# robocin/rSoccer

Hardware: AMD Instinct MI355X
Metric: env-steps/sec (whole node), VSS-v0 3v3 @4096 envs, 1/2/4/8 GPU + CPU ref (higher is better)
Workload: dtype f32

## Files before the change

rsoccer_amd/csrc/rsx_api.hip:

```cpp
#include <hip/hip_runtime.h>

#include <cstdio>
#include <cmath>
#include <cstdlib>
#include <algorithm>
#include <cstring>
#include <string>
#include <vector>

#include "rsx.h"
#include "rsx_units.hpp"
#include "rsx_variants.hpp"

using namespace rsx;

namespace {

thread_local std::string g_err;

int fail(int code, const std::string& msg) { g_err = msg; return code; }

#define HIP_TRY(expr)                                                                      \
    do {                                                                                   \
        hipError_t _e = (expr);                                                            \
// ... 591 lines not shown
    RSX_ENTER(h);
    h->host_state_valid = false;
    launch_sim(h, (hipStream_t)stream);
    HIP_TRY(launch_status());
    return debug_finite(h, (hipStream_t)stream, "rsx_step_dev");
}

static int ensure_alt(rsx_sim* h) {
    if (h->d_state_alt) return RSX_OK;
    const size_t sbytes = (size_t)(h->P.state_dim + X_ROWS) * h->P.row_stride * sizeof(float);
    HIP_TRY(hipMalloc((void**)&h->alt_alloc, sbytes));
    h->d_state_alt = h->alt_alloc;
    HIP_TRY(hipMemset(h->d_state_alt, 0, sbytes));
    HIP_TRY(hipDeviceSynchronize());
    return RSX_OK;
}

int rsx_state_buffers(rsx_sim* h, float** current, float** other) {
    RSX_ENTER(h);
    if (!current || !other) return fail(RSX_ERR_ARG, "null argument");
    if (int rc = ensure_alt(h)) return rc;
    *current = h->d_state; *other = h->d_state_alt;
    h->host_state_cache = false; h->host_state_valid = false;
    return RSX_OK;
}

int rsx_step_dev_random(rsx_sim* h, int n, uint64_t seed, uint32_t first_tick, void* stream) {
    RSX_ENTER(h);
    if (n < 1) return fail(RSX_ERR_ARG, "n must be >= 1");
    if ((uint64_t)first_tick + (uint64_t)n > 0x7FFFFFFFull) return fail(RSX_ERR_ARG, "tick range exceeds 2^31");
    h->host_state_valid = false;
    for (int i = 0; i < n; ++i) launch_sim(h, (hipStream_t)stream, nullptr, (int)(first_tick + (uint32_t)i), seed);
    HIP_TRY(launch_status());
    return debug_finite(h, (hipStream_t)stream, "rsx_step_dev_random");
}

int rsx_step_dev_flip(rsx_sim* h, void* stream) {
    RSX_ENTER(h);
    {
        hipStreamCaptureStatus cs = hipStreamCaptureStatusNone;
        if (hipStreamIsCapturing((hipStream_t)stream, &cs) != hipSuccess) (void)hipGetLastError();
        else if (cs != hipStreamCaptureStatusNone) return fail(RSX_ERR_STATE, "rsx_step_dev_flip cannot be captured (the buffer roles are host state); capture rsx_step_dev instead");
    }
    if (int rc = ensure_alt(h)) return rc;
    h->host_state_valid = false;
    launch_sim(h, (hipStream_t)stream, h->d_state_alt);
    HIP_TRY(launch_status());
    std::swap(h->d_state, h->d_state_alt);
    return debug_finite(h, (hipStream_t)stream, "rsx_step_dev_flip");
}

int rsx_reset_dev(rsx_sim* h, const float* ball_dev, const float* blue_dev, const float* yellow_dev,
                  const uint8_t* env_mask_dev, void* stream) {
    RSX_ENTER(h);
    if (!ball_dev || (h->P.n_blue && !blue_dev) || (h->P.n_yellow && !yellow_dev)) return fail(RSX_ERR_ARG, "null placement array");
    h->host_state_valid = false;
    const int B = h->P.num_envs;
    rsx_launch(reset_dev_kernel, dim3((B + 255) / 256), dim3(256), 0, (hipStream_t)stream, h->d_state, ball_dev, blue_dev,
                       yellow_dev, env_mask_dev, B, h->P.row_stride, h->P.state_dim + X_ROWS, h->M.rs, h->P.n_blue, h->P.n_yellow, (float)h->M.field[6]);
    HIP_TRY(launch_status());
    return RSX_OK;
}

int rsx_task_attach(rsx_sim* h, int task, uint64_t seed, uint64_t env_id_base, int max_episode_steps) {
    RSX_ENTER(h);
    if (h->P.task != RSX_TASK_NONE) return fail(RSX_ERR_STATE, "a task is already attached");
    if (env_id_base > 0xFFFFFFFFull || env_id_base + (uint64_t)h->P.num_envs > 0x100000000ull)
        return fail(RSX_ERR_ARG, "env_id_base + num_envs exceeds 2^32 (global env ids are 32-bit)");
    Params P = h->P;
    if (derive_task(task, seed, env_id_base, max_episode_steps, h->M, P))
        return fail(RSX_ERR_ARG, "task does not match the simulator (VSS_V0: VSS, n_blue >= 1; STATIC_DEFENDERS: SSL 1vN; DRIBBLING: SSL 1v4; CONTESTED: SSL 1v1; PASS_ENDURANCE: SSL 2v0; SCRIMMAGE: SSL)");
    if (P.obs_dim > 64) return fail(RSX_ERR_ARG, "observation wider than 64 floats is not supported");
    if (task >= RSX_TASK_SSL_DRIBBLING && task <= RSX_TASK_SSL_PASS_ENDURANCE && h->L != 8)
        return fail(RSX_ERR_ARG, "this task runs with 8 lanes per env only (unset RSX_LANES_PER_ENV)");
    const size_t B = (size_t)P.num_envs, S = (size_t)P.row_stride;
    const size_t n_aux = align_up((size_t)aux_rows(P.n_robots) * S * sizeof(float));
    if (n_aux >= ((size_t)1 << 32) || B * (size_t)P.obs_dim * sizeof(float) >= ((size_t)1 << 32))
        return fail(RSX_ERR_ARG, "num_envs too large for a fused task: the per-env scalar arena or the observation array would reach 4 GB (see rsx.h, limits)");
    const size_t n_obs = align_up(B * P.obs_dim * sizeof(float));
    const size_t n_flags = align_up(3 * B);
    const size_t n_act = align_up(B * h->M.act_dim * sizeof(float));
    const size_t n_met = align_up((size_t)TICK_SLOT_WORD0 * 4 + ((size_t)grid_for(h) + (B + 63) / 64) * sizeof(uint32_t));
    const size_t n_slots = align_up((size_t)MSLOTS * RSX_METRICS * sizeof(unsigned long long));
    const bool pc = !std::getenv("RSX_NO_PCACHE") && h->L == 8 && P.num_envs <= RSX_PCACHE_MAX_ENVS && P.n_sub > 0 &&
                    task == RSX_TASK_SSL_STATIC_DEFENDERS && h->NR == 7;
    const size_t n_pc = pc ? align_up((size_t)2 * (3 * (P.n_robots + 1) + 1) * B * sizeof(float)) : 0;
    const size_t n_pcs = pc && std::getenv("RSX_PCACHE_STATS") ? align_up(2 * sizeof(unsigned long long)) : 0;
    const size_t total = n_aux + 2 * n_obs + n_flags + n_act + n_met + n_slots + n_pc + n_pcs;
    HIP_TRY(hipMalloc((void**)&h->arena_task, total));
    HIP_TRY(hipMemset(h->arena_task, 0, total));
    h->arena_task_bytes = total; h->pcache_bytes = n_pc;
    char* p = h->arena_task;
    h->d_aux = (float*)p; p += n_aux;
    h->d_obs = (float*)p; p += n_obs;
    h->d_final_obs = (float*)p; p += n_obs;
    h->d_flags = (uint8_t*)p; p += n_flags;
    h->d_actions = (float*)p; p += n_act;
    h->d_metrics = (unsigned long long*)p; p += n_met;
    h->d_mslots = (unsigned long long*)p; p += n_slots;
    if (n_pc) {
        h->d_pcache = (float*)p; p += n_pc;
        HIP_TRY(hipMemset(h->d_pcache, 0xFF, n_pc));
    }
    if (n_pcs) h->d_pcstats = (unsigned long long*)p;
    HIP_TRY(hipMemset(h->d_aux + (size_t)ROW_EPISODE * S, 0xFF, B * sizeof(uint32_t)));
    h->P = P;
    h->epl = false;
    h->big = false; h->quad = false;
    if ((task == RSX_TASK_SSL_SCRIMMAGE || task == RSX_TASK_SSL_SCRIMMAGE_CROWDED) && h->NR == 22 && h->L == 32) {
        h->big = P.num_envs >= RSX_BIG_MIN_ENVS;
        const char* lay = std::getenv("RSX_LAYOUT");
        const size_t rows = (size_t)std::max(P.state_dim + X_ROWS, aux_rows(P.n_robots));
        const bool fits = rows * (size_t)P.row_stride * sizeof(float) < ((size_t)1 << 31) && P.n_sub > 0 && P.n_blue == 11;
        const int quad_min = task == RSX_TASK_SSL_SCRIMMAGE ? RSX_QUAD_MIN_ENVS : RSX_QUAD_MIN_ENVS_CROWDED;
        h->quad = fits && (lay ? std::strcmp(lay, "quad") == 0 : (quad_min > 0 && P.num_envs >= quad_min));
    }
    const bool fixed_ssl = task == RSX_TASK_SSL_DRIBBLING || task == RSX_TASK_SSL_CONTESTED || task == RSX_TASK_SSL_PASS_ENDURANCE;
    if ((task == RSX_TASK_VSS_V0 && h->NR == 6 && h->L == 8) || (task == RSX_TASK_SSL_STATIC_DEFENDERS && h->NR == 7 && h->L == 8) || fixed_ssl) {
        const char* lay = std::getenv("RSX_LAYOUT");
        if (lay && std::strcmp(lay, "epl") == 0) h->epl = true;
        else if (lay && std::strcmp(lay, "lanes") == 0) h->epl = false;
        else h->epl = P.num_envs >= (task == RSX_TASK_VSS_V0 ? RSX_EPL_MIN_ENVS : task == RSX_TASK_SSL_STATIC_DEFENDERS ? RSX_EPL_MIN_ENVS_SSL
                                     : task == RSX_TASK_SSL_DRIBBLING ? 49152 : 32768);
        const size_t rows = (size_t)std::max(P.state_dim + X_ROWS, aux_rows(P.n_robots));
        if (rows * (size_t)P.row_stride * sizeof(float) >= ((size_t)1 << 31) || (size_t)P.num_envs * P.obs_dim * sizeof(float) >= ((size_t)1 << 31)) h->epl = false;
    }
    if (h->d_phys) h->epl = h->big = h->quad = false;
    h->task_ready = false;
    h->tick_dev = false;
    h->tick_slots = step_grid(h, MODE_STEP);
    h->tick_slots_alloc = std::max(h->tick_slots, grid_for(h) + (P.num_envs + 63) / 64);
    HIP_TRY(hipDeviceSynchronize());
    return RSX_OK;
}

int rsx_drop_pending_hip_error(void) { return (int)hipGetLastError(); }

int rsx_task_reseed(rsx_sim* h, uint64_t seed, void* stream) {
    RSX_ENTER_TASK(h);
    hipStream_t s = (hipStream_t)stream;
    hipStreamCaptureStatus cs = hipStreamCaptureStatusNone;
    if (hipStreamIsCapturing(s, &cs) != hipSuccess) (void)hipGetLastError();
    else if (cs != hipStreamCaptureStatusNone) return fail(RSX_ERR_STATE, "rsx_task_reseed changes host state (seed, step counter) and cannot be captured");
    HIP_TRY(hipMemsetAsync(h->arena_task, 0, h->arena_task_bytes, s));
    if (h->d_pcache) HIP_TRY(hipMemsetAsync(h->d_pcache, 0xFF, h->pcache_bytes, s));
    HIP_TRY(hipMemsetAsync(h->d_aux + (size_t)ROW_EPISODE * h->P.row_stride, 0xFF, (size_t)h->P.num_envs * sizeof(uint32_t), s));
    h->P.key0 = (uint32_t)seed; h->P.key1 = (uint32_t)(seed >> 32);
    h->tick = 0; h->P.tick_base = 0;
    h->task_ready = false;
    return RSX_OK;
}

int rsx_task_enable_capture(rsx_sim* h, void* stream) {
    RSX_ENTER_TASK(h);
    (void)hipGetLastError();
    if (h->tick_dev) return RSX_OK;
    hipStream_t s = (hipStream_t)stream;
    hipStreamCaptureStatus cs = hipStreamCaptureStatusNone;
    if (hipStreamIsCapturing(s, &cs) != hipSuccess) (void)hipGetLastError();
    else if (cs != hipStreamCaptureStatusNone)
        return fail(RSX_ERR_STATE, "rsx_task_enable_capture must be called BEFORE the capture begins (it writes the step counter once; a captured write would reset it on every replay)");
    tick_fill(h, 0, h->tick_slots_alloc, h->tick, 0, s);
    HIP_TRY(launch_status());
    h->tick_dev = true;
    h->host_state_cache = false; h->host_state_valid = false;
    return RSX_OK;
}

// ... 479 lines not shown
```

rsoccer_amd/csrc/rsx_kernels.hpp:

```cpp
#pragma once
#include <hip/hip_runtime.h>
#include <type_traits>

#include "rsx_math.hpp"
#include "rsx_params.hpp"
#include "rsx_body.hpp"
#include "rsx_phys.hpp"

namespace rsx {

constexpr int ROW_REWARD = 0, ROW_PREV_POT = 1, ROW_EP_RET = 2, ROW_STEPS = 3, ROW_EPISODE = 4,
              ROW_INFO = 5 , ROW_OU = 15 ;
__host__ __device__ constexpr int aux_rows(int n_robots) { return ROW_OU + 2 * n_robots; }

struct Buffers {
    float* state;
    float* aux;
    float* obs;
    float* final_obs;
    uint8_t* flags;
    const float* cmds;
    const float* actions;
    unsigned long long* metrics;
    unsigned long long* mslots;
    float* pcache;
    unsigned long long* pcstats;
#ifdef RSX_TIMING
    unsigned long long* dbg;
#endif
};

template <int L>
struct Shared {
    float4 A[64];
    float4 Bq[64];
    float4 Cq[64];
    float Dq[64];
    float W[64];
    float2 F[64];
    alignas(16) float X[64], Y[64];
    float x0[64 / L][12];
    float2 draws[64 / L][L < 16 ? 16 : L];
    uint32_t ep[64];
#ifdef RSX_TIMING
    unsigned long long* dbg;
#endif
};

#define RSX_RARE_B(KIND, bit, c) (((KIND) == RSX_KIND_SSL || (6 & (bit))) ? __builtin_expect(!!(c), 0) : !!(c))

typedef uint32_t ix_t;
__device__ __forceinline__ float& at_byte(float* base, const ix_t off) { return *reinterpret_cast<float*>(reinterpret_cast<char*>(base) + off); }
__device__ __forceinline__ const float& at_byte(const float* base, const ix_t off) { return *reinterpret_cast<const float*>(reinterpret_cast<const char*>(base) + off); }

template <int L>
struct LaneMap {
    static constexpr int G = 64 / L;
    static constexpr bool EM = L == 8;
    static __device__ __forceinline__ int slot(const int j, const int g) { return EM ? g * L + j : j * G + g; }
    static __device__ __forceinline__ int body(const int lane) { return EM ? lane % L : lane / G; }
    static __device__ __forceinline__ int env(const int lane) { return EM ? lane / L : lane % G; }
};
template <int L>
__device__ __forceinline__ unsigned long long env_lane_mask(const int g) {
    constexpr int G = 64 / L;
    if (LaneMap<L>::EM) return ((1ull << L) - 1ull) << (g * L);
    unsigned long long m = 0;
#pragma unroll
    for (int j = 0; j < L; ++j) m |= 1ull << (j * G);
    return m << g;
}

__device__ __forceinline__ void load_coefs(const Params& P, const float* __restrict__ phys, const int e, EnvCoef& cf) {
    const float* const rows = phys + PHYS_HDR_FLOATS + (size_t)NPHYS * (size_t)P.row_stride;
    const ix_t B4 = (ix_t)4 * (ix_t)P.row_stride, off = (ix_t)4 * (ix_t)e;
#pragma unroll
    for (int i = 0; i < NCOEF; ++i) cf.c[i] = at_byte(rows, off + (ix_t)i * B4);
}
__device__ __forceinline__ void phys_redraw(const Params& P, float* __restrict__ phys, const int e, const uint32_t env_id,
                                            const uint32_t episode, const bool writer, EnvCoef& cf) {
    const PhysHeader* const hd = reinterpret_cast<const PhysHeader*>(phys);
    const uint32_t mask = hd->mask;
    if (mask == 0u) return;
    const size_t S = (size_t)P.row_stride;
    float* const raw = phys_raw(phys);
    float v[NPHYS];
#pragma unroll
    for (int p = 0; p < NPHYS; ++p) {
        if ((mask >> p) & 1u) {
            const u32x4 u = philox4x32(env_id, episode, (uint32_t)p, DOM_PHYS, P.key0, P.key1);
            v[p] = hd->lo[p] + (hd->hi[p] - hd->lo[p]) * u01(u.x);
        } else {
            v[p] = raw[(size_t)p * S + e];
        }
    }
    derive_coefs(hd->kind, hd->ts_ms, v, cf.c);
    if (writer) {
        float* const co = phys_coef(phys, S);
#pragma unroll
        for (int p = 0; p < NPHYS; ++p)
            if ((mask >> p) & 1u) raw[(size_t)p * S + e] = v[p];
#pragma unroll
        for (int i = 0; i < NCOEF; ++i) co[(size_t)i * S + e] = cf.c[i];
    }
}

template <int KIND, int L, class CF = LitCoef<KIND>>
__device__ __forceinline__ bool vss_sweep_loop(const Params& P, Body& o, const int N, const int g, const bool is_ball,
                                               const bool ball_low, const Shared<L>& sh, bool& wallp, const float2 fo, const CF& cf = CF{}) {
    using K = KC<KIND>;
    constexpr int G = 64 / L;
    constexpr uint32_t T_RR = __builtin_bit_cast(uint32_t, K::rs_rr2) - 1u;
    constexpr uint32_t T_RB = __builtin_bit_cast(uint32_t, K::rs_rb2) - 1u;
    unsigned todo = 0;
#pragma unroll 4
    for (int j = 0; j <= N; ++j) {
        const float4 oj = sh.A[LaneMap<L>::slot(j, g)];
        const bool rb = is_ball || j == N;
        const float dx = oj.x - o.x, dy = oj.y - o.y;
        const uint32_t u = __float_as_uint(fma_(dx, dx, dy * dy)) - 1u;
        todo |= ((u < (rb ? T_RB : T_RR)) & (!rb | ball_low)) ? 1u << j : 0u;
    }
    if (todo == 0) return false;
    const bool v2w = K::wall_aware && __ballot(!is_ball && at_wall<KIND>(P, o.x, o.y)) != 0ull;
    bool deep = false;
    float avx = 0.0f, avy = 0.0f, apx = 0.0f, apy = 0.0f, aw = 0.0f;
    const Body snap = o;
    const float lever = is_ball ? K::r_ball : K::r_robot;
// ... 113 lines not shown
        float dx = ob.x - o.x, dy = ob.y - o.y;
        float nx = 0.0f, ny = 0.0f, pen = -1.0f;
        bool mouth = false, touch = false;
        constexpr float NEAR2 = 0.13f * 0.13f;
        const float d2 = fma_(dx, dx, dy * dy);
        if (ball_low && d2 < NEAR2) {
            float lx = fma_(dx, o.c, dy * o.s), ly = fma_(dy, o.c, -(dx * o.s));
            if (fabsf(ly) < K::half_kw && lx > 0.0f) {
                mouth = true; pen = K::dck_rb - lx; nx = o.c; ny = o.s; touch = pen > 0.0f;
            } else {
                if (d2 < K::rs_rb2 && d2 > 0.0f) {
                    float d = sqrtf(d2), inv = 1.0f / d;
                    nx = dx * inv; ny = dy * inv; pen = K::rs_rb - d; touch = true;
                }
            }
        }
        float4 r0 = make_float4(0.0f, 0.0f, 0.0f, 0.0f), r1 = make_float4(0.0f, 0.0f, 0.0f, 0.0f);
        float dws = 0.0f;
        if (touch) {
            touched |= pen > K::pen2;
            got = true;
            const float dvx = ob.z - o.vx, dvy = ob.w - o.vy;
            float vn = fma_(dvx, nx, dvy * ny);
            if (vn < 0.0f) {
                const float omb = sh.W[LaneMap<L>::slot(N, g)];
                float q = cf.ope_rb() * vn * cf.w_rb_r(); avx = fma_(q, nx, avx); avy = fma_(q, ny, avy);
                const float wsum = fma_(omb, K::r_ball, o.om * (mouth ? K::dck : K::r_robot));
                const float vt = fma_(dvy, nx, -(dvx * ny)) - wsum;
                const float lim = q * cf.mu_rb();
                const float ft = clampf(vt * cf.kt_rb_r(), lim, -lim);
                avx = fma_(-ft, ny, avx); avy = fma_(ft, nx, avy);
                float qb = cf.ope_rb() * vn * cf.w_rb_b();
                const float limb = qb * cf.mu_rb();
                const float ftb = clampf(vt * cf.kt_rb_b(), limb, -limb);
                r0.x = fma_(-ftb, ny, qb * nx); r0.y = fma_(ftb, nx, qb * ny); dws = ftb * K::spin_c; fl |= 1;
            }
            float pc = K::beta * pen * cf.w_rb_r();
            apx = fma_(-pc, nx, apx); apy = fma_(-pc, ny, apy);
            float pb = K::beta * pen * cf.w_rb_b(); r0.z = pb * nx; r0.w = pb * ny; fl |= 2;
        }
        if (first) {
            o.ir = mouth && pen > -K::ir_tol;
            if (o.ir) {
                if (o.kick_x > 0.0f || o.kick_z > 0.0f) {
                    fl |= 4 | 8;
                    r1.y = o.vx + o.kick_x * o.c; r1.z = o.vy + o.kick_x * o.s; r1.w = o.kick_z;
                } else if (o.drib) {
                    float hx = o.x + K::dck_rb * o.c, hy = o.y + K::dck_rb * o.s;
                    float cvx = (hx - ob.x) * P.drib_gain, cvy = (hy - ob.y) * P.drib_gain;
                    float m2 = cvx * cvx + cvy * cvy;
                    if (m2 > K::drib_vmax2) { float sc = K::drib_vmax / sqrtf(m2); cvx = cvx * sc; cvy = cvy * sc; }
                    fl |= 4;
                    r1.y = (o.vx - o.om * K::dck_rb * o.s) + cvx;
                    r1.z = (o.vy + o.om * K::dck_rb * o.c) + cvy;
                }
            }
        }
        r1.x = __int_as_float(fl);
        if (fl) { sh.Bq[lane] = r0; sh.Cq[lane] = r1; sh.Dq[lane] = dws; }
    }
    const unsigned long long wrote = __ballot(fl != 0);
    wave_sync();
    if (is_ball) {
        unsigned long long todo = L <= 32 ? (env_lane_mask<L>(g) & wrote) : wrote;
        while (todo) {
            const int lj = __builtin_ctzll(todo);
            todo &= todo - 1;
            const float4 r1 = sh.Cq[lj];
            const float4 r0 = sh.Bq[lj];
            const int flj = __float_as_int(r1.x);
            if (flj & 1) { avx = avx - r0.x; avy = avy - r0.y; aw = aw + sh.Dq[lj]; }
            if (flj & 2) { apx = apx + r0.z; apy = apy + r0.w; got = true; }
            if (flj & 4) { bo.ovr = true; bo.okick = (flj & 8) != 0; bo.ovx = r1.y; bo.ovy = r1.z; bo.ovz = r1.w; }
        }
    }
    if (got) {
        o.vx = o.vx + avx; o.vy = o.vy + avy;
        o.x = o.x + apx; o.y = o.y + apy;
        if (is_ball) o.om = o.om + aw;
    }
    return touched;
}

template <int KIND, int L, int NR, class CF = LitCoef<KIND>>
__device__ __forceinline__ void physics(const Params& P, Body& o, const int b, const int g,
                                        const bool live, Shared<L>& sh, const CF& cf = CF{}) {
    using K = KC<KIND>;
    constexpr int G = 64 / L;
    const int N = NR ? NR : P.n_robots;
    const bool is_robot = live && b < N;
    const bool is_ball = live && b == N;
    const int lane = LaneMap<L>::slot(b, g);

    if (is_ball) ball_step_friction(P, o, cf);
#ifdef RSX_TIMING_SUB
    unsigned long long tsA = 0, tsB = 0, tsC = 0, ts0 = 0, ts1 = 0, ts2 = 0;
#endif

    for (int sub = 0; sub < P.n_sub; ++sub) {
#ifdef RSX_TIMING_SUB
        ts0 = __builtin_readcyclecounter();
#endif
        if (is_robot) {
            actuate_robot<KIND>(P, o, cf);
            o.th = advance_heading(P, o.om, o.th);
            rotate_heading(o.om * P.h, o.c, o.s);
        }
        if (RSX_RARE_B(KIND, 1, is_ball && (o.z > 0.0f || o.vz > 0.0f))) ball_flight(P, o, K::e_ground, K::vz_min);
        o.x = fma_(o.vx, P.h, o.x);
        o.y = fma_(o.vy, P.h, o.y);
#ifdef RSX_TIMING_SUB
        ts1 = __builtin_readcyclecounter();
#endif

        const unsigned long long lowm = __ballot(is_ball && o.z < K::robot_h);
        bool ball_low = ((lowm >> (LaneMap<L>::slot(N, g))) & 1ull) != 0;
        bool active = is_robot || is_ball;
        BallOverride bo{false, false, 0.0f, 0.0f, 0.0f};
        for (int sweep = 0;; ++sweep) {
            float2 fo = float2{0.0f, 0.0f};
            if (active) {
                sh.A[lane] = make_float4(o.x, o.y, o.vx, o.vy);
                sh.W[lane] = o.om;
                sh.X[g * L + b] = o.x; sh.Y[g * L + b] = o.y;
            }
            wave_sync();
            auto publish_held = [&]() {
                if constexpr (K::held) { fo = held_axes<KIND>(P, o.x, o.y, is_robot); sh.F[lane] = fo; }
            };
            bool deep = false;
            bool wallp = false;

            if (KIND == RSX_KIND_VSS) {
                if (active) {
                    if (NR) {
                        constexpr uint32_t T_RR = __builtin_bit_cast(uint32_t, K::rs_rr2) - 1u;
                        constexpr uint32_t T_RB = __builtin_bit_cast(uint32_t, K::rs_rb2) - 1u;
                        uint32_t u[NR + 1];
                        if constexpr (K::held) overlap_keys_packed<NR + 1, L>(sh, g, o.x, o.y, u, publish_held);
                        else overlap_keys_packed<NR + 1, L>(sh, g, o.x, o.y, u);
                        uint32_t um = u[0];
#pragma unroll
                        for (int j = 1; j < NR; ++j) um = min(um, u[j]);
                        const bool any = ((um < (is_ball ? T_RB : T_RR)) & (!is_ball | ball_low)) | ((u[NR] < T_RB) & ball_low);
                        if (RSX_RARE_B(KIND, 2, any)) {
                            unsigned todo = 0;
                            const uint32_t thr_r = is_ball ? T_RB : T_RR;
#pragma unroll
                            for (int j = NR; j >= 0; --j) {
                                if (j == NR) asm("v_cmp_gt_u32_e32 vcc, %2, %1\n\tv_addc_co_u32_e32 %0, vcc, %0, %0, vcc" : "+v"(todo) : "v"(u[j]), "s"(T_RB) : "vcc");
                                else asm("v_cmp_gt_u32_e32 vcc, %2, %1\n\tv_addc_co_u32_e32 %0, vcc, %0, %0, vcc" : "+v"(todo) : "v"(u[j]), "v"(thr_r) : "vcc");
                            }
                            if (!ball_low) todo = is_ball ? 0u : (todo & ~(1u << NR));
                            const bool v2w = K::wall_aware && __ballot(is_robot && at_wall<KIND>(P, o.x, o.y)) != 0ull;
                            float avx = 0.0f, avy = 0.0f, apx = 0.0f, apy = 0.0f, aw = 0.0f;
                            const float lever = is_ball ? K::r_ball : K::r_robot;
                            int jn = __builtin_ctz(todo);
                            todo &= todo - 1;
                            float4 nxt = sh.A[LaneMap<L>::slot(jn, g)];
                            float nxw = sh.W[LaneMap<L>::slot(jn, g)];
                            float2 nxf = sh.F[LaneMap<L>::slot(jn, g)];
                            for (;;) {
                                const int j = jn;
                                const float4 oj = nxt;
                                const float wj = nxw;
                                const float2 fj = nxf;
                                const bool more = todo != 0;
                                if (more) {
                                    jn = __builtin_ctz(todo);
                                    todo &= todo - 1;
                                    nxt = sh.A[LaneMap<L>::slot(jn, g)];
                                    nxw = sh.W[LaneMap<L>::slot(jn, g)];
                                    nxf = sh.F[LaneMap<L>::slot(jn, g)];
                                }
                                const float dx = oj.x - o.x, dy = oj.y - o.y;
                                const float d2 = fma_(dx, dx, dy * dy);
                                const bool rb = is_ball || j == NR;
                                contact_response<KIND>(P, o, oj, d2, rb ? K::rs_rb : K::rs_rr, rb ? cf.ope_rb() : cf.ope_rr(),
                                                       is_ball ? cf.w_rb_b() : (j == NR ? cf.w_rb_r() : K::w_rr),
                                                       is_ball ? cf.kt_rb_b() : (j == NR ? cf.kt_rb_r() : K::kt_rr),
                                                       rb ? cf.mu_rb() : cf.mu_rr(), is_ball ? K::spin_c : 0.0f,
                                                       fma_(wj, j == NR ? K::r_ball : K::r_robot, o.om * lever), K::beta, K::pen2, !rb, v2w,
                                                       avx, avy, apx, apy, aw, deep, wallp, fo, fj);
                                if (!more) break;
                            }
                            o.vx = o.vx + avx; o.vy = o.vy + avy;
                            o.x = o.x + apx; o.y = o.y + apy;
                            if (is_ball) o.om = o.om + aw;
                        }
                    } else {
                        publish_held();
                        deep = vss_sweep_loop<KIND, L>(P, o, N, g, is_ball, ball_low, sh, wallp, fo, cf);
                    }
                }
            } else {
                deep = ssl_sweep<KIND, L, NR>(P, o, N, g, lane, is_robot && active, is_ball && active, ball_low, sweep == 0, sh, bo, wallp, cf);
            }
            const unsigned long long dmask = __ballot(deep);
            if (sweep == 3 || !RSX_RARE_B(KIND, 2, dmask != 0)) break;
            bool again = (L == 64 ? dmask : (dmask & env_lane_mask<L>(g))) != 0;
            if (sweep >= 1) {
                const unsigned long long wmask = __ballot(wallp);
                again = again && (L == 64 ? wmask : (wmask & env_lane_mask<L>(g))) != 0;
            }
            active = active && again;
            if (sweep >= 1 && !__any(active)) break;
            wave_sync();
        }
        if (KIND == RSX_KIND_SSL && bo.ovr) {
            o.vx = bo.ovx; o.vy = bo.ovy; o.om = 0.0f;
            if (bo.okick && bo.ovz > 0.0f) o.vz = bo.ovz;
        }

#ifdef RSX_TIMING_SUB
        ts2 = __builtin_readcyclecounter();
#endif
        if (KIND == RSX_KIND_SSL ? __any(near_walls<KIND>(P, o.x, o.y)) : (is_robot || is_ball)) {
            const float vx0 = o.vx, vy0 = o.vy;
            int hit = 0;
            if constexpr (KIND == RSX_KIND_VSS) {
                const float rb = is_ball ? K::r_ball : K::r_robot, eb = is_ball ? cf.e_wb() : cf.e_wr();
                walls<KIND, true>(P, rb, eb, o.x, o.y, o.vx, o.vy, hit);
                if (RSX_RARE_B(KIND, 2, (is_ball && (hit & 3)) || (hit & 8))) {
                    if (hit & 8) post_response(P, rb, eb, o.x, o.y, o.vx, o.vy, hit);
                    if (is_ball && (hit & 3)) ball_wall_spin<KIND>(hit, vx0, vy0, o.vx, o.vy, o.om, cf.mu_wb(), cf.ope_wb());
                }
            } else {
            walls<KIND>(P, is_ball ? K::r_ball : K::r_robot, is_ball ? cf.e_wb() : cf.e_wr(), o.x, o.y, o.vx, o.vy, hit);
            if (RSX_RARE_B(KIND, 2, is_ball && hit)) ball_wall_spin<KIND>(hit, vx0, vy0, o.vx, o.vy, o.om, cf.mu_wb(), cf.ope_wb());
            }
        }
        wave_sync();
#ifdef RSX_TIMING
        if (threadIdx.x == 0 && sh.dbg) sh.dbg[(size_t)(8 + sub) * gridDim.x + blockIdx.x] = __builtin_readcyclecounter();
#endif
#ifdef RSX_TIMING_SUB
        if (sub >= 1) { const unsigned long long t3 = __builtin_readcyclecounter(); tsA += ts1 - ts0; tsB += ts2 - ts1; tsC += t3 - ts2; }
#endif
    }
#ifdef RSX_TIMING_SUB
    if (threadIdx.x == 0 && sh.dbg) {
        sh.dbg[(size_t)15 * gridDim.x + blockIdx.x] = tsA; sh.dbg[(size_t)16 * gridDim.x + blockIdx.x] = tsB; sh.dbg[(size_t)17 * gridDim.x + blockIdx.x] = tsC;
    }
#endif
}

struct RawBody { float v0, v1, v2, v3, v4, v5, ir , w[4]; };

template <int KIND>
__device__ __forceinline__ RawBody load_raw(const Params& P, const float* __restrict__ st, int e,
                                            int b, bool is_robot, bool is_ball) {
    constexpr int RS = ModelD<KIND>::rs;
    const ix_t B4 = (ix_t)4 * (ix_t)P.row_stride, e4 = (ix_t)4 * (ix_t)e;
    RawBody r{};
    if (is_robot || is_ball) {
        const int row0 = is_ball ? 0 : 5 + RS * b;
        const int row5 = is_ball ? P.state_dim : row0 + 5;
        const ix_t i0 = (ix_t)row0 * B4 + e4;
        r.v0 = at_byte(st, i0); r.v1 = at_byte(st, i0 + B4); r.v2 = at_byte(st, i0 + 2 * B4); r.v3 = at_byte(st, i0 + 3 * B4); r.v4 = at_byte(st, i0 + 4 * B4);
        r.v5 = at_byte(st, (ix_t)row5 * B4 + e4);
    }
    if (KIND == RSX_KIND_SSL) {
        if (is_robot || is_ball) r.ir = at_byte(st, (ix_t)(is_ball ? P.state_dim + 1 : 5 + RS * b + 6) * B4 + e4);
        if (is_robot) {
            const ix_t i7 = (ix_t)(5 + RS * b + 7) * B4 + e4;
#pragma unroll
            for (int i = 0; i < 4; ++i) r.w[i] = at_byte(st, i7 + (ix_t)i * B4);
        }
    } else if (is_ball) {
        r.ir = at_byte(st, (ix_t)(P.state_dim + 1) * B4 + e4);
    }
    return r;
}

template <int KIND>
__device__ __forceinline__ void interpret_body(const RawBody& r, bool is_robot, bool is_ball, Body& o,
                                               float& th_deg, float& om_deg, float w[4]) {
    using K = KC<KIND>;
    o = Body{};
    th_deg = 0.0f; om_deg = 0.0f;
    w[0] = w[1] = w[2] = w[3] = 0.0f;
    o.x = r.v0; o.y = r.v1; o.vx = r.v3; o.vy = r.v4;
    if (is_robot) {
        th_deg = r.v2; om_deg = r.v5;
        if (KIND == RSX_KIND_SSL) {
            o.ir = r.ir != 0.0f;
#pragma unroll
            for (int i = 0; i < 4; ++i) w[i] = r.w[i];
        }
// ... 586 lines not shown
```

rsoccer_amd/csrc/rsx_task_step_body.inc:

```
    constexpr bool HOT = MODE != MODE_ROLLOUT;
    Params P = P_;
    Buffers bufs = bufs_;
    if (HOT) {
        RSX_UNPACK_HOT(P);
        bufs.state = hp_state; bufs.aux = hp_aux; bufs.actions = hp_in; bufs.flags = hp_flags;
    }
    const int n_steps_arg = hp_n_steps & RSX_N_STEPS_MASK;
    constexpr int mode = MODE == MODE_ROLLOUT ? MODE_STEP : MODE;
    const int n_steps = MODE == MODE_ROLLOUT ? n_steps_arg : 1;
    const bool tick_dev = __builtin_expect((hp_n_steps & RSX_TICK_DEV) != 0, 0);
    using K = KC<KIND>;
    using T = TC<TASK>;
    constexpr int G = 64 / L;
    constexpr int ID = T::info_dim;
    constexpr int AD = T::act_dim;
    __shared__ Shared<L> sh;
    constexpr bool PC = !PHYS && MODE == MODE_STEP && L == 8 && TASK == RSX_TASK_SSL_STATIC_DEFENDERS && NR == 7;
    if constexpr (PC) {
        if (__builtin_expect(bufs.pcache != nullptr && (int)blockIdx.x >= hp_per_xcd * 8, 0)) {
            const StepTick th = step_tick(tick_dev, P, bufs, 1u);
            if (th.ok) placement_helper<KIND, L, TASK, (PC ? NR : 1)>(P, bufs, (int)blockIdx.x - hp_per_xcd * 8, th.t, sh);
            return;
        }
    }
    StepTick tk{0u, true};
    if (MODE == MODE_STEP || MODE == MODE_ROLLOUT) {
        tk = step_tick(tick_dev, P, bufs, (uint32_t)n_steps);
        if (__builtin_expect(!tk.ok, 0)) return;
    }
    const uint32_t tick0 = tk.t;
    const int lane = threadIdx.x;
    const int b = LaneMap<L>::body(lane), g = LaneMap<L>::env(lane);
    const int tile = tile_of_block(HOT ? hp_per_xcd : (int)(gridDim.x >> 3));
    const int e = tile * G + g;
    const int N = NR ? NR : P.n_robots;
    const bool live = e < P.num_envs;
    const bool is_robot = live && b < N, is_ball = live && b == N;
    const size_t B = (size_t)P.num_envs;
    const uint32_t env_id = P.env_id_base + (uint32_t)e;
    constexpr int OD_C = NR == 0 ? 0
        : TASK == RSX_TASK_VSS_V0 ? 4 + 6 * NR
        : TASK == RSX_TASK_SSL_STATIC_DEFENDERS ? 4 + 8 + 2 * (NR - 1)
        : TASK == RSX_TASK_SSL_SCRIMMAGE ? 2 + 2 * NR
        : TASK == RSX_TASK_SSL_DRIBBLING ? 21 : TASK == RSX_TASK_SSL_CONTESTED ? 14 : 16;
    const int OD = OD_C ? OD_C : P.obs_dim;
#define auxe(ROW) at_byte(bufs.aux, (ix_t)(ROW) * ((ix_t)4 * (ix_t)P.row_stride) + (ix_t)4 * (ix_t)e)

#ifdef RSX_TIMING
#define RSX_STAMP(i) do { if (lane == 0) bufs.dbg[(size_t)(i) * gridDim.x + blockIdx.x] = __builtin_readcyclecounter(); } while (0)
#else
#define RSX_STAMP(i) do {} while (0)
#endif
#ifdef RSX_TIMING
    if (lane == 0) { sh.dbg = bufs.dbg; bufs.dbg[(size_t)13 * gridDim.x + blockIdx.x] = __builtin_amdgcn_s_memrealtime(); }
#endif
    RSX_STAMP(0);
    Body o; float od, wd, wheels[4];
    const RawBody raw = load_raw<KIND>(P, bufs.state, e, b, is_robot, is_ball);
    constexpr bool CODE_PF = !PHYS && KIND == RSX_KIND_VSS && MODE == MODE_STEP;
    uint32_t code_touch = 0;
    if (CODE_PF) {
        unsigned long long pc;
        asm volatile("s_getpc_b64 %0" : "=s"(pc));
        code_touch = __builtin_nontemporal_load(reinterpret_cast<const uint32_t*>(reinterpret_cast<const char*>(pc) + 128u * (unsigned)lane));
    }
    std::conditional_t<PHYS, EnvCoef, LitCoef<KIND>> cf{};
    if constexpr (PHYS) if (live) load_coefs(P, phys, e, cf);
    int steps = 0; uint32_t episode = 0;
    if (live) {
        steps = __float_as_int(auxe(ROW_STEPS));
        episode = __float_as_uint(auxe(ROW_EPISODE));
    }
    float ou0 = 0.0f, ou1 = 0.0f;
    if (TASK == RSX_TASK_VSS_V0 && is_robot && b >= 1) {
        ou0 = auxe(ROW_OU + 2 * b); ou1 = auxe(ROW_OU + 2 * b + 1);
    }
    float info[10] = {0, 0, 0, 0, 0, 0, 0, 0, 0, 0};
    float prev_pot = 0.0f, ep_ret = 0.0f;
    if (is_ball) {
#pragma unroll
        for (int i = 0; i < ID; ++i)
            if (!(TASK == RSX_TASK_VSS_V0 && (i == 0 || i >= 4))) info[i] = auxe(ROW_INFO + i);
        prev_pot = auxe(ROW_PREV_POT);
        if (TASK != RSX_TASK_VSS_V0) ep_ret = auxe(ROW_EP_RET);
    }
    const bool counts_steps = (MODE == MODE_STEP || MODE == MODE_ROLLOUT) && blockIdx.x == 0 && lane == 0;
    unsigned long long steps_before = 0;
    if (counts_steps) steps_before = bufs.metrics[0];
    float reward = 0.0f; int term = 0, trunc = 0;
    bool success = false;
    bool against = false;
    bool was_reset = false;
    const bool fed = MODE == MODE_STEP && bufs.actions != nullptr;
    float act[AD];
#pragma unroll
    for (int i = 0; i < AD; ++i) act[i] = 0.0f;
    if (TASK == RSX_TASK_SSL_SCRIMMAGE) {
        if (fed && is_robot) {
#pragma unroll
            for (int i = 0; i < AD; ++i) act[i] = at_byte(bufs.actions, (ix_t)4 * (((ix_t)e * (ix_t)N + (ix_t)b) * (ix_t)AD + (ix_t)i));
        }
    } else if (fed && is_robot && b == 0) {
#pragma unroll
        for (int i = 0; i < AD; ++i) act[i] = at_byte(bufs.actions, (ix_t)4 * ((ix_t)e * (ix_t)AD + (ix_t)i));
    }

    float pcx = 0.0f, pcy = 0.0f, pcth = 0.0f;
    uint32_t ptag = 0u;
    bool pc_on = false;
    if constexpr (PC) {
        pc_on = bufs.pcache != nullptr;
        if (pc_on && (is_robot || is_ball)) {
            constexpr int NBD = (PC ? NR : 1) + 1;
            const float* const pr = bufs.pcache + (size_t)((tick0 + 1u) & 1u) * (size_t)pcache_rows<NBD>() * B;
            pcx = pr[(size_t)(0 * NBD + b) * B + e]; pcy = pr[(size_t)(1 * NBD + b) * B + e]; pcth = pr[(size_t)(2 * NBD + b) * B + e];
            ptag = __float_as_uint(pr[(size_t)(3 * NBD) * B + e]);
        }
    }

    StepDraw pre;
    if (MODE == MODE_STEP) pre = draw_for_step<KIND, TASK>(P, env_id, tick0, b, is_robot, fed);

    __builtin_amdgcn_s_waitcnt(0x0F70);
    if (CODE_PF) asm volatile("" :: "v"(code_touch));
    interpret_body<KIND>(raw, is_robot, is_ball, o, od, wd, wheels);
    RSX_STAMP(1);

    for (int it = 0; it < n_steps; ++it) {
        bool ended;
        const float obs_ts = prev_pot;
        if (mode == 2) {
            const bool flagged = live && bufs.flags[2 * B + e] != 0;
            if (flagged) {
                episode += 1; steps = 0; ou0 = 0.0f; ou1 = 0.0f;
                if constexpr (PHYS) phys_redraw(P, phys, e, env_id, episode, b == 0, cf);
                if (is_ball) {
#pragma unroll
                    for (int i = 0; i < 10; ++i) info[i] = 0.0f;
#pragma unroll
                    for (int i = 0; i < ID; ++i) auxe(ROW_INFO + i) = 0.0f;
                    ep_ret = 0.0f; prev_pot = 0.0f;
                }
            }
            if (flagged) write_obs<KIND, TASK>(P, bufs.obs + (size_t)e * OD, b, is_robot, is_ball, o.x, o.y, o.vx, o.vy, o.s, o.c, wd, o.ir, prev_pot);
            wave_sync();
            ended = false;
        } else if (mode == 1) {
            ended = live;
            episode += 1;
            if (is_ball) {
#pragma unroll
                for (int i = 0; i < 10; ++i) info[i] = 0.0f;
#pragma unroll
                for (int i = 0; i < ID; ++i) auxe(ROW_INFO + i) = 0.0f;
                ep_ret = 0.0f; prev_pot = 0.0f;
            }
        } else {
            const bool first_step = steps == 0;
            const uint32_t t = tick0 + (uint32_t)it;
            if (is_ball && first_step) {
#pragma unroll
                for (int i = 0; i < 10; ++i) info[i] = 0.0f;
                ep_ret = 0.0f;
            }
            const float lastx = o.x, lasty = o.y;

            float q[8] = {0, 0, 0, 0, 0, 0, 0, 0};
            const StepDraw dr = MODE == MODE_STEP ? pre : draw_for_step<KIND, TASK>(P, env_id, t, b, is_robot, fed);
            if (TASK == RSX_TASK_VSS_V0) {
                if (is_robot) {
                    float a0, a1;
                    if (b == 0) {
                        if (fed) { a0 = act[0]; a1 = act[1]; }
                        else { a0 = dr.v[0]; a1 = dr.v[1]; }
                    } else {
                        ou0 = (ou0 + P.ou_theta_dt * (0.0f - ou0)) + P.ou_sig_sqdt * dr.v[0];
                        ou1 = (ou1 + P.ou_theta_dt * (0.0f - ou1)) + P.ou_sig_sqdt * dr.v[1];
                        a0 = ou0; a1 = ou1;
                    }
                    q[0] = vss_wheel(a0); q[1] = vss_wheel(a1);
                }
            } else if (TASK == RSX_TASK_SSL_SCRIMMAGE) {
                if (is_robot) {
                    float a[4];
#pragma unroll
                    for (int i = 0; i < 4; ++i) a[i] = fed ? act[i] : dr.v[i];
                    q[1] = a[0] * T::max_v; q[2] = a[1] * T::max_v; q[3] = a[2] * 10.0f;
                    q[5] = a[3] > 0.9f ? 5.0f : 0.0f;
                }
            } else {
                if (is_robot && b == 0) {
                    float a[5] = {0, 0, 0, 0, 0};
#pragma unroll
                    for (int i = 0; i < AD; ++i) a[i] = fed ? act[i] : dr.v[i];
                    ssl_agent_commands<TASK>(a, o.s, o.c, q);
                }
                if (TASK == RSX_TASK_SSL_PASS_ENDURANCE && is_robot && b == 1) q[7] = 1.0f;
            }
            if (is_robot) robot_targets<KIND>(P, o, q);

            RSX_STAMP(2);
            physics<KIND, L, NR>(P, o, b, g, live, sh, cf);
            RSX_STAMP(3);
            if (MODE == MODE_STEP && KIND == RSX_KIND_SSL) {
                typedef const __attribute__((address_space(4))) uint32_t* kw_t;
                constexpr size_t KOFF = RSX_PARAMS_KERNARG_OFFSET;
                static_assert(sizeof(Params) % 4 == 0 && KOFF % 4 == 0, "parameter block in dwords");
                kw_t pk = (kw_t)__builtin_amdgcn_kernarg_segment_ptr() + KOFF / 4;
                asm volatile("" : "+s"(pk));
                struct Words { uint32_t w[sizeof(Params) / 4]; } raw;
#pragma unroll
                for (size_t i = 0; i < sizeof(Params) / 4; ++i) raw.w[i] = pk[i];
                P = __builtin_bit_cast(Params, raw);
                RSX_UNPACK_HOT(P);
            }

            if (is_robot) {
                od = o.th; wd = o.om * K::rad2deg;
                if (KIND == RSX_KIND_SSL) wheel_speeds<KIND>(P, o, wheels);
                o.om = wd * K::deg2rad;
                sincos_f32(o.th * K::deg2rad, o.s, o.c);
            } else if (is_ball) {
                o.z = (K::r_ball + o.z) - K::r_ball;
            }
            write_obs<KIND, TASK>(P, bufs.obs + (size_t)e * OD, b, is_robot, is_ball, o.x, o.y, o.vx, o.vy, o.s, o.c, wd, o.ir, obs_ts);
            if (is_robot && b == 0) {
                float* xr = sh.x0[g];
                xr[0] = o.x; xr[1] = o.y;
                if (TASK == RSX_TASK_VSS_V0) { xr[2] = o.vx; xr[3] = o.vy; xr[4] = q[0]; xr[5] = q[1]; }
                else if (TASK == RSX_TASK_SSL_STATIC_DEFENDERS || TASK == RSX_TASK_SSL_CONTESTED) {
                    xr[6] = lastx; xr[7] = lasty;
                    xr[8] = wheels[0]; xr[9] = wheels[1]; xr[10] = wheels[2]; xr[11] = wheels[3];
                }
            } else if (is_robot) {
                float* xr = sh.x0[g];
                if (TASK == RSX_TASK_SSL_DRIBBLING) xr[1 + b] = (fabsf(o.vx) > 0.05f || fabsf(o.vy) > 0.05f) ? 1.0f : 0.0f;
                if (TASK == RSX_TASK_SSL_CONTESTED && b == 1) xr[2] = (fabsf(o.vx) > 0.1f || fabsf(o.vy) > 0.1f) ? 1.0f : 0.0f;
                if (TASK == RSX_TASK_SSL_PASS_ENDURANCE && b == 1) { xr[2] = o.x; xr[3] = o.y; xr[4] = o.ir ? 1.0f : 0.0f; }
            }
            wave_sync();
            if (is_ball) {
                const float* xr = sh.x0[g];
                task_reward<KIND, TASK>(P, xr, o.x, o.y, lastx, lasty, first_step, prev_pot, info, reward, term, success, against);
                ep_ret = ep_ret + reward;
            }
            steps += 1;
            trunc = steps >= P.max_steps;
            const unsigned long long endm = __ballot(is_ball && (term | trunc));
            ended = live && ((endm >> (LaneMap<L>::slot(N, g))) & 1ull) != 0;
            if (is_ball) {
#pragma unroll
                for (int i = 0; i < ID; ++i)
                    if (!(TASK == RSX_TASK_VSS_V0 && (i == 0 || i >= 4)) || term || first_step) auxe(ROW_INFO + i) = info[i];
                auxe(ROW_REWARD) = reward;
                if (MODE == MODE_STEP) { bufs.flags[(ix_t)e] = (uint8_t)term; bufs.flags[(ix_t)P.num_envs + (ix_t)e] = (uint8_t)trunc; }
                else { bufs.flags[e] = (uint8_t)term; bufs.flags[B + e] = (uint8_t)trunc; }
            }
        }

        RSX_STAMP(4);
        if (RSX_RARE_B(KIND, 4, __any(ended))) {
            if (ended && mode == 0) {
                write_obs<KIND, TASK>(P, bufs.final_obs + (size_t)e * OD, b, is_robot, is_ball, o.x, o.y, o.vx, o.vy, o.s, o.c, wd, o.ir, obs_ts);
            }
            if (ended && mode == 0) episode += 1;
            if (KIND == RSX_KIND_VSS) {
                if (ended && is_ball && mode == 0) {
                    unsigned long long* const ms = metric_slot(bufs);
                    atomicAdd(&ms[1], 1ull);
                    if (info[4] > 0.0f) atomicAdd(&ms[2], 1ull);
                    if (info[5] > 0.0f) atomicAdd(&ms[3], 1ull);
                    atomicAdd(&ms[4], (unsigned long long)__float2ll_rn(vss_episode_return(info) * 1048576.0f));
                    atomicAdd(&ms[5], (unsigned long long)steps);
                    if (trunc && !term) atomicAdd(&ms[6], 1ull);
                }
            } else if (mode == 0) {
                static_assert(KIND == RSX_KIND_VSS || L >= 6, "metrics fan-out needs 6 lanes per env");
                uint32_t* const mv = reinterpret_cast<uint32_t*>(sh.x0[g]);
                if (ended && is_ball) {
                    unsigned long long inc[6];
                    inc[0] = 1ull;
                    inc[1] = success ? 1ull : 0ull;
                    inc[2] = against ? 1ull : 0ull;
                    inc[3] = (unsigned long long)__float2ll_rn(ep_ret * 1048576.0f);
                    inc[4] = (unsigned long long)steps;
                    inc[5] = (trunc && !term) ? 1ull : 0ull;
#pragma unroll
                    for (int k = 0; k < 6; ++k) { mv[2 * k] = (uint32_t)inc[k]; mv[2 * k + 1] = (uint32_t)(inc[k] >> 32); }
                }
                wave_sync();
                if (ended && b < 6) {
                    const unsigned long long v = (unsigned long long)mv[2 * b] | ((unsigned long long)mv[2 * b + 1] << 32);
                    if (v) atomicAdd(&metric_slot(bufs)[1 + b], v);
                }
            }
            RSX_STAMP(15);
            const bool hit = PC && pc_on && ended && ptag == episode;
            const bool place = ended && !hit;
            const bool any_place = !PC || __any(place);
            if (any_place) {
                if (place) place_predraw<TASK, L>(P, env_id, episode, b, sh.draws[g]);
                wave_sync();
            }
            RSX_STAMP(16);
            float4 pz = make_float4(0.0f, 0.0f, 0.0f, 0.0f);
            if (TASK == RSX_TASK_SSL_SCRIMMAGE) {
                if (ended && (is_robot || is_ball)) {
                    const u32x4 u = philox4x32(env_id, episode, (uint32_t)b, DOM_PLACE, P.key0, P.key1);
                    const float jx = u01(u.x) * 2.0f - 1.0f, jy = u01(u.y) * 2.0f - 1.0f;
                    if (is_ball) pz = make_float4(P.sc_jb * jx, P.sc_jb * jy, 0.0f, 0.0f);
                    else pz = make_float4(P.sc_sx * ((float)(b % 6) - 2.5f) + P.sc_j * jx,
                                          P.sc_sy * ((float)(b / 6) - 1.5f) + P.sc_j * jy, 360.0f * u01(u.z), 0.0f);
                }
            } else if ((TASK == RSX_TASK_VSS_V0 || TASK == RSX_TASK_SSL_STATIC_DEFENDERS) && MODE != MODE_ROLLOUT) {
                if (any_place && place) pz = place_env_parallel<TASK, L, NR>(P, N, env_id, episode, b, g, is_robot, sh.A, sh.draws[g]);
                if (hit) pz = make_float4(pcx, pcy, pcth, 0.0f);
                if (PC && pc_on && bufs.pcstats && ended && is_ball) atomicAdd(&bufs.pcstats[hit ? 0 : 1], 1ull);
            } else {
                if (ended && is_ball) place_env<TASK, L>(P, N, env_id, episode, g, sh.A, sh.draws[g]);
                wave_sync();
                if (ended && (is_robot || is_ball)) pz = sh.A[LaneMap<L>::slot(b, g)];
            }
            RSX_STAMP(17);
            if (ended) {
                steps = 0; ou0 = 0.0f; ou1 = 0.0f; was_reset = true;
                if constexpr (PHYS) phys_redraw(P, phys, e, env_id, episode, b == 0, cf);
                if (TASK >= RSX_TASK_SSL_DRIBBLING) prev_pot = 0.0f;
                if (is_robot || is_ball) {
                    o = Body{};
                    o.x = pz.x; o.y = pz.y;
                    od = pz.z; wd = 0.0f;
                    wheels[0] = wheels[1] = wheels[2] = wheels[3] = 0.0f;
                    if (is_robot) { o.th = od; sincos_f32(o.th * K::deg2rad, o.s, o.c); }
                }
                write_obs<KIND, TASK>(P, bufs.obs + (size_t)e * OD, b, is_robot, is_ball, o.x, o.y, o.vx, o.vy, o.s, o.c, wd, 0, 0.0f);
            }
            wave_sync();
            RSX_STAMP(18);
        }

        wave_sync();
    }

    RSX_STAMP(5);
    if (mode != 2) store_body<KIND>(P, bufs.state, e, b, is_robot, is_ball, o, od, wd, wheels, P.n_sub != 0 || was_reset);
    if (live && b == 0) {
        auxe(ROW_STEPS) = __int_as_float(steps);
        auxe(ROW_EPISODE) = __uint_as_float(episode);
    }
    if (TASK == RSX_TASK_VSS_V0 && is_robot && b >= 1) {
        auxe(ROW_OU + 2 * b) = ou0; auxe(ROW_OU + 2 * b + 1) = ou1;
    }
    if (is_ball) {
        auxe(ROW_PREV_POT) = prev_pot;
        if (TASK != RSX_TASK_VSS_V0) auxe(ROW_EP_RET) = ep_ret;
#undef auxe
    }
    if (counts_steps) bufs.metrics[0] = steps_before + (unsigned long long)P.num_envs * (unsigned long long)n_steps;
    RSX_STAMP(6);
#ifdef RSX_TIMING
    __builtin_amdgcn_s_waitcnt(0x0F70);
    RSX_STAMP(7);
    if (lane == 0) bufs.dbg[(size_t)14 * gridDim.x + blockIdx.x] = __builtin_amdgcn_s_memrealtime();
#endif
```

Baseline: 435.6 million.

## Enable placement cache for VSS, add single-contact fast path, fan out VSS metrics

Extends the reset-placement cache (previously limited to SSL static-defenders) to VSS-v0 with 6 robots, so that episode resets can reuse precomputed placements instead of redrawing them. It also adds a wave-uniform fast path in the collision response for the case where every lane has at most one contact, skipping the software-pipelined loop. VSS metric accumulation in step mode now goes through the lane fan-out path, which spreads the 64-bit atomics across six lanes instead of issuing them serially from the ball lane. Timing-only counters and a code-prefetch offset macro are added behind debug defines. In exchange the change adds an arena allocation and cache bookkeeping for VSS, plus a ballot on every collision sweep.

```diff
diff --git a/rsoccer_amd/csrc/rsx_api.hip b/rsoccer_amd/csrc/rsx_api.hip
--- a/rsoccer_amd/csrc/rsx_api.hip
+++ b/rsoccer_amd/csrc/rsx_api.hip
@@ -697,8 +697,13 @@
     const size_t n_act = align_up(B * h->M.act_dim * sizeof(float));
     const size_t n_met = align_up((size_t)TICK_SLOT_WORD0 * 4 + ((size_t)grid_for(h) + (B + 63) / 64) * sizeof(uint32_t));
     const size_t n_slots = align_up((size_t)MSLOTS * RSX_METRICS * sizeof(unsigned long long));
+#ifdef RSX_LOO_PCACHE
+    const bool pc_vss = false;
+#else
+    const bool pc_vss = task == RSX_TASK_VSS_V0 && h->NR == 6;
+#endif
     const bool pc = !std::getenv("RSX_NO_PCACHE") && h->L == 8 && P.num_envs <= RSX_PCACHE_MAX_ENVS && P.n_sub > 0 &&
-                    task == RSX_TASK_SSL_STATIC_DEFENDERS && h->NR == 7;
+                    ((task == RSX_TASK_SSL_STATIC_DEFENDERS && h->NR == 7) || pc_vss);
     const size_t n_pc = pc ? align_up((size_t)2 * (3 * (P.n_robots + 1) + 1) * B * sizeof(float)) : 0;
     const size_t n_pcs = pc && std::getenv("RSX_PCACHE_STATS") ? align_up(2 * sizeof(unsigned long long)) : 0;
     const size_t total = n_aux + 2 * n_obs + n_flags + n_act + n_met + n_slots + n_pc + n_pcs;
diff --git a/rsoccer_amd/csrc/rsx_kernels.hpp b/rsoccer_amd/csrc/rsx_kernels.hpp
--- a/rsoccer_amd/csrc/rsx_kernels.hpp
+++ b/rsoccer_amd/csrc/rsx_kernels.hpp
@@ -44,6 +44,7 @@
     uint32_t ep[64];
 #ifdef RSX_TIMING
     unsigned long long* dbg;
+    uint32_t cls_depth, cls_flags;
 #endif
 };
 
@@ -323,7 +324,7 @@
     return touched;
 }
 
-template <int KIND, int L, int NR, class CF = LitCoef<KIND>>
+template <int KIND, int L, int NR, bool LONE = false, class CF = LitCoef<KIND>>
 __device__ __forceinline__ void physics(const Params& P, Body& o, const int b, const int g,
                                         const bool live, Shared<L>& sh, const CF& cf = CF{}) {
     using K = KC<KIND>;
@@ -393,27 +394,13 @@
                                 else asm("v_cmp_gt_u32_e32 vcc, %2, %1\n\tv_addc_co_u32_e32 %0, vcc, %0, %0, vcc" : "+v"(todo) : "v"(u[j]), "v"(thr_r) : "vcc");
                             }
                             if (!ball_low) todo = is_ball ? 0u : (todo & ~(1u << NR));
+#ifdef RSX_TIMING
+                            if (sh.dbg) atomicMax(&sh.cls_depth, (uint32_t)__builtin_popcount(todo));
+#endif
                             const bool v2w = K::wall_aware && __ballot(is_robot && at_wall<KIND>(P, o.x, o.y)) != 0ull;
                             float avx = 0.0f, avy = 0.0f, apx = 0.0f, apy = 0.0f, aw = 0.0f;
                             const float lever = is_ball ? K::r_ball : K::r_robot;
-                            int jn = __builtin_ctz(todo);
-                            todo &= todo - 1;
-                            float4 nxt = sh.A[LaneMap<L>::slot(jn, g)];
-                            float nxw = sh.W[LaneMap<L>::slot(jn, g)];
-                            float2 nxf = sh.F[LaneMap<L>::slot(jn, g)];
-                            for (;;) {
-                                const int j = jn;
-                                const float4 oj = nxt;
-                                const float wj = nxw;
-                                const float2 fj = nxf;
-                                const bool more = todo != 0;
-                                if (more) {
-                                    jn = __builtin_ctz(todo);
-                                    todo &= todo - 1;
-                                    nxt = sh.A[LaneMap<L>::slot(jn, g)];
-                                    nxw = sh.W[LaneMap<L>::slot(jn, g)];
-                                    nxf = sh.F[LaneMap<L>::slot(jn, g)];
-                                }
+                            auto respond_to = [&](const int j, const float4 oj, const float wj, const float2 fj) {
                                 const float dx = oj.x - o.x, dy = oj.y - o.y;
                                 const float d2 = fma_(dx, dx, dy * dy);
                                 const bool rb = is_ball || j == NR;
@@ -423,7 +410,37 @@
                                                        rb ? cf.mu_rb() : cf.mu_rr(), is_ball ? K::spin_c : 0.0f,
                                                        fma_(wj, j == NR ? K::r_ball : K::r_robot, o.om * lever), K::beta, K::pen2, !rb, v2w,
                                                        avx, avy, apx, apy, aw, deep, wallp, fo, fj);
-                                if (!more) break;
+                            };
+#ifdef RSX_LOO_STRAIGHT
+                            const bool single = false;
+#else
+                            const bool single = LONE && __ballot((todo & (todo - 1u)) != 0u) == 0ull;
+#endif
+                            if (__builtin_expect(single, 1)) {
+                                const int j = __builtin_ctz(todo);
+                                respond_to(j, sh.A[LaneMap<L>::slot(j, g)], sh.W[LaneMap<L>::slot(j, g)], sh.F[LaneMap<L>::slot(j, g)]);
+                            } else {
+                                int jn = __builtin_ctz(todo);
+                                todo &= todo - 1;
+                                float4 nxt = sh.A[LaneMap<L>::slot(jn, g)];
+                                float nxw = sh.W[LaneMap<L>::slot(jn, g)];
+                                float2 nxf = sh.F[LaneMap<L>::slot(jn, g)];
+                                for (;;) {
+                                    const int j = jn;
+                                    const float4 oj = nxt;
+                                    const float wj = nxw;
+                                    const float2 fj = nxf;
+                                    const bool more = todo != 0;
+                                    if (more) {
+                                        jn = __builtin_ctz(todo);
+                                        todo &= todo - 1;
+                                        nxt = sh.A[LaneMap<L>::slot(jn, g)];
+                                        nxw = sh.W[LaneMap<L>::slot(jn, g)];
+                                        nxf = sh.F[LaneMap<L>::slot(jn, g)];
+                                    }
+                                    respond_to(j, oj, wj, fj);
+                                    if (!more) break;
+                                }
                             }
                             o.vx = o.vx + avx; o.vy = o.vy + avy;
                             o.x = o.x + apx; o.y = o.y + apy;
@@ -446,6 +463,9 @@
             }
             active = active && again;
             if (sweep >= 1 && !__any(active)) break;
+#ifdef RSX_TIMING
+            if (threadIdx.x == 0 && sh.dbg) sh.cls_flags |= 1u;
+#endif
             wave_sync();
         }
         if (KIND == RSX_KIND_SSL && bo.ovr) {
diff --git a/rsoccer_amd/csrc/rsx_task_step_body.inc b/rsoccer_amd/csrc/rsx_task_step_body.inc
--- a/rsoccer_amd/csrc/rsx_task_step_body.inc
+++ b/rsoccer_amd/csrc/rsx_task_step_body.inc
@@ -15,7 +15,12 @@
     constexpr int ID = T::info_dim;
     constexpr int AD = T::act_dim;
     __shared__ Shared<L> sh;
-    constexpr bool PC = !PHYS && MODE == MODE_STEP && L == 8 && TASK == RSX_TASK_SSL_STATIC_DEFENDERS && NR == 7;
+#ifdef RSX_LOO_PCACHE
+    constexpr bool PC_VSS = false;
+#else
+    constexpr bool PC_VSS = TASK == RSX_TASK_VSS_V0 && NR == 6;
+#endif
+    constexpr bool PC = !PHYS && MODE == MODE_STEP && L == 8 && ((TASK == RSX_TASK_SSL_STATIC_DEFENDERS && NR == 7) || PC_VSS);
     if constexpr (PC) {
         if (__builtin_expect(bufs.pcache != nullptr && (int)blockIdx.x >= hp_per_xcd * 8, 0)) {
             const StepTick th = step_tick(tick_dev, P, bufs, 1u);
@@ -52,17 +57,20 @@
 #define RSX_STAMP(i) do {} while (0)
 #endif
 #ifdef RSX_TIMING
-    if (lane == 0) { sh.dbg = bufs.dbg; bufs.dbg[(size_t)13 * gridDim.x + blockIdx.x] = __builtin_amdgcn_s_memrealtime(); }
+    if (lane == 0) { sh.dbg = bufs.dbg; sh.cls_depth = 0u; sh.cls_flags = 0u; bufs.dbg[(size_t)13 * gridDim.x + blockIdx.x] = __builtin_amdgcn_s_memrealtime(); }
 #endif
     RSX_STAMP(0);
     Body o; float od, wd, wheels[4];
     const RawBody raw = load_raw<KIND>(P, bufs.state, e, b, is_robot, is_ball);
     constexpr bool CODE_PF = !PHYS && KIND == RSX_KIND_VSS && MODE == MODE_STEP;
+#ifndef RSX_PF_SHIFT
+#define RSX_PF_SHIFT 0u
+#endif
     uint32_t code_touch = 0;
     if (CODE_PF) {
         unsigned long long pc;
         asm volatile("s_getpc_b64 %0" : "=s"(pc));
-        code_touch = __builtin_nontemporal_load(reinterpret_cast<const uint32_t*>(reinterpret_cast<const char*>(pc) + 128u * (unsigned)lane));
+        code_touch = __builtin_nontemporal_load(reinterpret_cast<const uint32_t*>(reinterpret_cast<const char*>(pc) + RSX_PF_SHIFT + 128u * (unsigned)lane));
     }
     std::conditional_t<PHYS, EnvCoef, LitCoef<KIND>> cf{};
     if constexpr (PHYS) if (live) load_coefs(P, phys, e, cf);
@@ -200,7 +208,7 @@
             if (is_robot) robot_targets<KIND>(P, o, q);
 
             RSX_STAMP(2);
-            physics<KIND, L, NR>(P, o, b, g, live, sh, cf);
+            physics<KIND, L, NR, MODE == MODE_STEP>(P, o, b, g, live, sh, cf);
             RSX_STAMP(3);
             if (MODE == MODE_STEP && KIND == RSX_KIND_SSL) {
                 typedef const __attribute__((address_space(4))) uint32_t* kw_t;
@@ -264,7 +272,12 @@
                 write_obs<KIND, TASK>(P, bufs.final_obs + (size_t)e * OD, b, is_robot, is_ball, o.x, o.y, o.vx, o.vy, o.s, o.c, wd, o.ir, obs_ts);
             }
             if (ended && mode == 0) episode += 1;
-            if (KIND == RSX_KIND_VSS) {
+#ifdef RSX_LOO_FANOUT
+            constexpr bool VSS_PLAIN = KIND == RSX_KIND_VSS;
+#else
+            constexpr bool VSS_PLAIN = KIND == RSX_KIND_VSS && MODE == MODE_ROLLOUT;
+#endif
+            if constexpr (VSS_PLAIN) {
                 if (ended && is_ball && mode == 0) {
                     unsigned long long* const ms = metric_slot(bufs);
                     atomicAdd(&ms[1], 1ull);
@@ -275,14 +288,14 @@
                     if (trunc && !term) atomicAdd(&ms[6], 1ull);
                 }
             } else if (mode == 0) {
-                static_assert(KIND == RSX_KIND_VSS || L >= 6, "metrics fan-out needs 6 lanes per env");
+                static_assert(L >= 6, "metrics fan-out needs 6 lanes per env");
                 uint32_t* const mv = reinterpret_cast<uint32_t*>(sh.x0[g]);
                 if (ended && is_ball) {
                     unsigned long long inc[6];
                     inc[0] = 1ull;
-                    inc[1] = success ? 1ull : 0ull;
-                    inc[2] = against ? 1ull : 0ull;
-                    inc[3] = (unsigned long long)__float2ll_rn(ep_ret * 1048576.0f);
+                    inc[1] = (KIND == RSX_KIND_VSS ? info[4] > 0.0f : success) ? 1ull : 0ull;
+                    inc[2] = (KIND == RSX_KIND_VSS ? info[5] > 0.0f : against) ? 1ull : 0ull;
+                    inc[3] = (unsigned long long)__float2ll_rn((KIND == RSX_KIND_VSS ? vss_episode_return(info) : ep_ret) * 1048576.0f);
                     inc[4] = (unsigned long long)steps;
                     inc[5] = (trunc && !term) ? 1ull : 0ull;
 #pragma unroll
@@ -337,6 +350,9 @@
             }
             wave_sync();
             RSX_STAMP(18);
+#ifdef RSX_TIMING
+            if (lane == 0 && mode == 0) sh.cls_flags |= 2u;
+#endif
         }
 
         wave_sync();
@@ -361,5 +377,8 @@
 #ifdef RSX_TIMING
     __builtin_amdgcn_s_waitcnt(0x0F70);
     RSX_STAMP(7);
-    if (lane == 0) bufs.dbg[(size_t)14 * gridDim.x + blockIdx.x] = __builtin_amdgcn_s_memrealtime();
-#endif
+    if (lane == 0) {
+        bufs.dbg[(size_t)14 * gridDim.x + blockIdx.x] = __builtin_amdgcn_s_memrealtime();
+        bufs.dbg[(size_t)19 * gridDim.x + blockIdx.x] = (unsigned long long)(sh.cls_depth | (sh.cls_flags << 8));
+    }
+#endif
```

After: 400.4 million. 8.1% lower.
